# c-zhou/oatk

Hardware: AMD Instinct MI355X
Metric: HiFi Gbases/s through syncasm (syncmer+syncerr) at k=1001 s=31 (higher is better)
Workload: dtype u64

## Files before the change

### oatk_amd/csrc/api.hip

```cpp
#include <hip/hip_runtime.h>
#include <rocprim/device/device_radix_sort.hpp>
#include <rocprim/device/device_scan.hpp>
#include <rocprim/device/device_transform.hpp>
#include <stdio.h>
#include <stdlib.h>
#include <string.h>
#include <time.h>
#include <sys/mman.h>
#include <mutex>
#include <string>
#include <thread>
#include <utility>
#include <vector>

#include "../../include/oatk_hip.h"
#include "devmem.hpp"
#include "common.hpp"
#include "scan_hpc.hpp"
#include "scan_syncmer.hpp"
#include "scan_syncmer_fast.hpp"
#include "kmer_hash.hpp"
#include "count.hpp"

struct oatk_hip_ctx {
    int device = 0;
    int n_cu = 256;
    hipStream_t stream = nullptr;
    std::string err;
    bool timing = false;
    hipEvent_t ev[OATK_T_COUNT_ + 1][2];
    bool ev_used[OATK_T_COUNT_ + 1];
    float ms[OATK_T_COUNT_];
    uint64_t hash_mask = ~0ULL;
    bool force_general = false;
    void *staging = nullptr;
    uint64_t staging_cap = 0;
    void *staging_raw = nullptr;
    uint64_t staging_raw_size = 0;
    bool ra_two_pass = false;
    int list_cap = 0;
    uint64_t import_reserve = 1u << 20;
    int ec_cap_t0 = 0, ec_cap_t1 = 0;

    const uint8_t *d_seq = nullptr;
    const uint64_t *d_off = nullptr;
    const uint32_t *d_len = nullptr;
    DevBuf in_seq, in_off, in_len;
    uint64_t n_reads = 0, seq_bytes = 0, sid0 = 0;
    int K = 0, S = 0;
    bool scanned = false, counted = false;
    bool slots_packed = false;

    DevBuf hoco_l, n_scm, n_nn, n_lrl, ho_rl, hoco_s, nbits;
    DevBuf nn_key, lrl_key, lrl_val, nn_key2, lrl_key2, lrl_val2;
    DevBuf raw_lo, raw_smer, raw_mpos, shard_cnt;
    uint32_t region_cap = 0;
    DevBuf counters;
    uint32_t nn_cap = 0, lrl_cap = 0;
    uint64_t n_occ = 0, tot_nn = 0, tot_lrl = 0, n_scm_total = 0;
    uint32_t retries = 0, collisions = 0;
    bool nn_sorted_in_2 = false, lrl_sorted_in_2 = false;

    DevBuf n_scm64, scm_off, pos_hash, pos_lo, pos_smer, pos_mpos, pos_kid;
    DevBuf key_hash, key_sorted, iota, perm, head, head_idx, newclus, clus_id, bad_head, tag, tmp_perm, flags, kloc, smer_sorted, slot_rec, scm_loc;
    DevBuf scm_h, scm_s, scm_cov, scm_occ_off, scm_occ;
    DevBuf tmp;
    struct EcState *ec = nullptr;
    struct ConsState *cons = nullptr;
    struct IngState *ing = nullptr;
    struct InfState *inf = nullptr;
    struct StatState *stat = nullptr;
    struct AgState *ag = nullptr;
    struct OvlState *ovl = nullptr;
    struct RaState *ra = nullptr;
    struct RcState *rc = nullptr;
    struct MultiState *multi = nullptr;
};

#define CK(call)                                                                                   \
    do {                                                                                           \
        hipError_t e_ = (call);                                                                    \
        if (e_ != hipSuccess) {                                                                    \
            ctx->err = std::string(#call) + ": " + hipGetErrorString(e_);                          \
            return OATK_E_NODEV;                                                                   \
        }                                                                                          \
    } while (0)
static bool debug_refuse(oatk_hip_ctx *ctx, int bit, const char *what)
{
    const char *e = getenv("OATK_DEBUG_REFUSE");
    if (!e || !(atoi(e) & bit)) return false;
    ctx->err = std::string(what) + ": refused on request (OATK_DEBUG_REFUSE)";
    return true;
}

static void t_begin(oatk_hip_ctx *ctx, int which)
{
    if (!ctx->timing) return;
    (void) hipEventRecord(ctx->ev[which][0], ctx->stream);
}
static void t_end(oatk_hip_ctx *ctx, int which)
{
    if (!ctx->timing) return;
    (void) hipEventRecord(ctx->ev[which][1], ctx->stream);
    ctx->ev_used[which] = true;
}
static void t_collect(oatk_hip_ctx *ctx, int first, int last)
{
    if (!ctx->timing) return;
    (void) hipStreamSynchronize(ctx->stream);
    for (int i = first; i <= last; ++i) {
        ctx->ms[i] = 0.f;
        if (ctx->ev_used[i]) (void) hipEventElapsedTime(&ctx->ms[i], ctx->ev[i][0], ctx->ev[i][1]);
        ctx->ev_used[i] = false;
    }
}

#include "api_prim.inc"
#include "api_ec.inc"
#include "api_graph.inc"
#include "api_cons.inc"
#include "api_ovl.inc"
#include "api_align.inc"
#include "api_ingest.inc"
#include "api_bam.inc"
#include "api_inflate.inc"
#include "api_stat.inc"
#include "api_multi.inc"
#include "api_multi_tail.inc"
#include "api_racov.inc"
#include "api_multiplex.inc"

static void staging_free(oatk_hip_ctx *ctx)
{
    if (!ctx->staging) return;
    if (ctx->staging_raw) { (void) hipHostUnregister(ctx->staging); munmap(ctx->staging_raw, ctx->staging_raw_size); }
    else (void) hipHostFree(ctx->staging);
    ctx->staging = ctx->staging_raw = nullptr, ctx->staging_cap = ctx->staging_raw_size = 0;
}

extern "C" {

int oatk_hip_abi_version(void) { return OATK_HIP_ABI_VERSION; }

int oatk_hip_device_count(void)
{
    int n = 0;
    if (hipGetDeviceCount(&n) != hipSuccess) return 0;
    return n;
}

int oatk_hip_max_k(void) { return 8192 - 16 * oatk::SYN_NT - 16 - 64; }

oatk_hip_ctx *oatk_hip_create(int device)
{
    int n = 0;
    if (hipGetDeviceCount(&n) != hipSuccess || device < 0 || device >= n) return nullptr;
    if (hipSetDevice(device) != hipSuccess) return nullptr;
    oatk_hip_ctx *ctx = new oatk_hip_ctx();
    ctx->device = device;
    { int cu = 0; if (hipDeviceGetAttribute(&cu, hipDeviceAttributeMultiprocessorCount, device) == hipSuccess && cu > 0) ctx->n_cu = cu; }
    if (hipStreamCreateWithFlags(&ctx->stream, hipStreamNonBlocking) != hipSuccess) { delete ctx; return nullptr; }
    for (int i = 0; i <= OATK_T_COUNT_; ++i) {
        (void) hipEventCreate(&ctx->ev[i][0]);
        (void) hipEventCreate(&ctx->ev[i][1]);
        ctx->ev_used[i] = false;
    }
    memset(ctx->ms, 0, sizeof(ctx->ms));
    return ctx;
}

void oatk_hip_destroy(oatk_hip_ctx *ctx)
{
    if (!ctx) return;
    (void) hipSetDevice(ctx->device);
    (void) hipStreamSynchronize(ctx->stream);
    ec_state_free(ctx);
    cons_state_free(ctx);
    ing_state_free(ctx);
    inf_state_free(ctx);
    stat_state_free(ctx);
    ag_state_free(ctx);
    ovl_state_free(ctx);
    ra_state_free(ctx);
    rc_state_free(ctx);
    multi_state_free(ctx);
    for (int i = 0; i <= OATK_T_COUNT_; ++i) {
        (void) hipEventDestroy(ctx->ev[i][0]);
        (void) hipEventDestroy(ctx->ev[i][1]);
    }
    staging_free(ctx);
    (void) hipStreamDestroy(ctx->stream);
    delete ctx;
}

int oatk_hip_mem_pool(oatk_hip_ctx *ctx, uint64_t warm_bytes)
{
    if (!ctx) return OATK_E_NODEV;
    { const char *e = getenv("OATK_POOL"); if (e && e[0] == '0') return OATK_OK; }
    CK(hipSetDevice(ctx->device));
    if (ctx->device < 0 || ctx->device >= 64) return OATK_E_ARG;
    ChunkPool *pl;
    {
        std::unique_lock<std::mutex> lk(g_pool_mu);
        pl = g_pool[ctx->device];
        if (!pl) {
            int vmm = 0;
            if (hipDeviceGetAttribute(&vmm, hipDeviceAttributeVirtualMemoryManagementSupported, ctx->device) != hipSuccess || !vmm) { (void) hipGetLastError(); return OATK_OK; }
            pl = new ChunkPool();
            pl->device = ctx->device;
            memset(&pl->prop, 0, sizeof(pl->prop));
            pl->prop.type = hipMemAllocationTypePinned;
            pl->prop.location.type = hipMemLocationTypeDevice;
            pl->prop.location.id = ctx->device;
            memset(&pl->acc, 0, sizeof(pl->acc));
            pl->acc.location = pl->prop.location;
            pl->acc.flags = hipMemAccessFlagsProtReadWrite;
            static bool at_exit = false;
            if (!at_exit) { at_exit = true; atexit(pools_end); }
            pl->on = true;
            g_pool[ctx->device] = pl;
        }
    }
    if (warm_bytes) pl->warm((size_t) warm_bytes);
    return OATK_OK;
}

const char *oatk_hip_last_error(oatk_hip_ctx *ctx) { return ctx? ctx->err.c_str() : "no device context"; }
void *oatk_hip_stream(oatk_hip_ctx *ctx) { return ctx? (void *) ctx->stream : nullptr; }
int oatk_hip_sync(oatk_hip_ctx *ctx)
{
    if (!ctx) return OATK_E_NODEV;
    CK(hipStreamSynchronize(ctx->stream));
    return OATK_OK;
}
int oatk_hip_set_timing(oatk_hip_ctx *ctx, int enable)
{
    if (!ctx) return OATK_E_NODEV;
    ctx->timing = enable != 0;
    return OATK_OK;
}
int oatk_hip_get_timing(oatk_hip_ctx *ctx, float *ms, int n)
{
    if (!ctx) return OATK_E_NODEV;
    for (int i = 0; i < n && i < OATK_T_COUNT_; ++i) ms[i] = ctx->ms[i];
    return OATK_OK;
}
int oatk_hip_debug_force_general(oatk_hip_ctx *ctx, int on)
{
    if (!ctx) return OATK_E_NODEV;
    ctx->force_general = on != 0;
    return OATK_OK;
}
int oatk_hip_debug_align_two_pass(oatk_hip_ctx *ctx, int on)
{
    if (!ctx) return OATK_E_NODEV;
    ctx->ra_two_pass = on != 0;
    return OATK_OK;
}
int oatk_hip_debug_list_cap(oatk_hip_ctx *ctx, int cap)
{
    if (!ctx) return OATK_E_NODEV;
    if (cap < 0 || cap > oatk::SYF_LIST) { ctx->err = "oatk_hip_debug_list_cap: 0 <= cap <= 128"; return OATK_E_ARG; }
    ctx->list_cap = cap;
    return OATK_OK;
}
int oatk_hip_debug_hash_mask(oatk_hip_ctx *ctx, uint64_t mask)
{
    if (!ctx) return OATK_E_NODEV;
    ctx->hash_mask = mask;
    return OATK_OK;
}

static void scan_reset_downstream(oatk_hip_ctx *ctx);

static int launch_scan_kernels(oatk_hip_ctx *ctx)
{
    using namespace oatk;
    const uint64_t n = ctx->n_reads;
    CK(hipMemsetAsync(ctx->counters.p, 0, 4 * sizeof(uint32_t), ctx->stream));
    CK(hipMemsetAsync(ctx->shard_cnt.p, 0, oatk::OATK_REC_SHARDS * sizeof(uint32_t), ctx->stream));
    HpcArgs h;
    h.seq = ctx->d_seq, h.off = ctx->d_off, h.len = ctx->d_len, h.sid0 = ctx->sid0;
    h.ho_rl = ctx->ho_rl.as<uint8_t>(), h.hoco_s = ctx->hoco_s.as<uint8_t>(), h.nbits = ctx->nbits.as<uint32_t>();
    h.hoco_l = ctx->hoco_l.as<uint32_t>(), h.n_nn = ctx->n_nn.as<uint32_t>(), h.n_lrl = ctx->n_lrl.as<uint32_t>();
    h.nn_key = ctx->nn_key.as<uint64_t>(), h.lrl_key = ctx->lrl_key.as<uint64_t>(), h.lrl_val = ctx->lrl_val.as<uint32_t>();
    h.nn_cap = ctx->nn_cap, h.lrl_cap = ctx->lrl_cap, h.counters = ctx->counters.as<uint32_t>();
    t_begin(ctx, OATK_T_HPC);
    h.n_reads = (uint32_t) n;
    constexpr int HPC_NW = 4;
    uint64_t hpc_grid = (uint64_t) ctx->n_cu * 8 * 8;
    { const char *ev = getenv("OATK_DEBUG_HPC_GRID"); if (ev && atoi(ev) > 0) hpc_grid = (uint64_t) atoi(ev); }
    if (hpc_grid * HPC_NW > n) hpc_grid = (n + HPC_NW - 1) / HPC_NW;
    unsigned hpc_dyn = 0;
    { const char *ev = getenv("OATK_DEBUG_HPC_LDS"); if (ev && atoi(ev) > 0) hpc_dyn = (unsigned) atoi(ev); }
    hipLaunchKernelGGL((hpc_pack_kernel<HPC_NW>), dim3((unsigned) (hpc_grid? hpc_grid : 1)), dim3(HPC_NW * OATK_WAVE), hpc_dyn, ctx->stream, h);
    t_end(ctx, OATK_T_HPC);

    SynArgs s;
    s.hoco_s = ctx->hoco_s.as<uint8_t>(), s.nbits = ctx->nbits.as<uint32_t>(), s.off = ctx->d_off;
    s.hoco_l = ctx->hoco_l.as<uint32_t>(), s.n_nn = ctx->n_nn.as<uint32_t>(), s.sid0 = ctx->sid0;
    s.K = ctx->K, s.S = ctx->S, s.want_n = 0, s.n_scm = ctx->n_scm.as<uint32_t>(), s.list_cap = ctx->list_cap? ctx->list_cap : SYF_LIST;
    s.rec_hash = nullptr, s.rec_lo = ctx->raw_lo.as<uint64_t>(), s.rec_smer = ctx->raw_smer.as<uint64_t>();
    s.rec_mpos = ctx->raw_mpos.as<uint32_t>(), s.region_cap = ctx->region_cap, s.shard_cnt = ctx->shard_cnt.as<uint32_t>();
    const bool small = ctx->K + 8 * SYN_NT + 8 + 64 <= 4096;
    const int fast_ring = ctx->force_general? 0 : syncmer_fast_ring(ctx->K, ctx->S);
    t_begin(ctx, OATK_T_SYNCMER);
    if (fast_ring == 4096) {
        const dim3 g((unsigned) n), b(SYN_NT);
        unsigned dyn = 0;
        { const char *ev = getenv("OATK_DEBUG_SYNCMER_LDS"); if (ev && atoi(ev) > 0) dyn = (unsigned) atoi(ev); }
#define OATK_SYF_SWITCH(S31) switch ((-(ctx->K - ctx->S)) & 7) { \
            case 0: OATK_SYF_LAUNCH(S31, 0); break; case 1: OATK_SYF_LAUNCH(S31, 1); break; case 2: OATK_SYF_LAUNCH(S31, 2); break; \
            case 3: OATK_SYF_LAUNCH(S31, 3); break; case 4: OATK_SYF_LAUNCH(S31, 4); break; case 5: OATK_SYF_LAUNCH(S31, 5); break; \
            case 6: OATK_SYF_LAUNCH(S31, 6); break; default: OATK_SYF_LAUNCH(S31, 7); break; }
        const bool two_waves = ctx->K - ctx->S < 1024 && getenv("OATK_DEBUG_SYNCMER_NT256") == nullptr;
#define OATK_SYF_LAUNCH(S31, SH) do { if (two_waves) hipLaunchKernelGGL((syncmer_fast_kernel<2048, S31, 128, SH>), g, dim3(128), dyn, ctx->stream, s); \
                                      else hipLaunchKernelGGL((syncmer_fast_kernel<4096, S31, SYN_NT, SH>), g, b, dyn, ctx->stream, s); } while (0)
        if (ctx->S == 31) OATK_SYF_SWITCH(true) else OATK_SYF_SWITCH(false)
#undef OATK_SYF_SWITCH
#undef OATK_SYF_LAUNCH
    }
    else if (small) hipLaunchKernelGGL((syncmer_kernel<8, 4096, false>), dim3((unsigned) n), dim3(SYN_NT), 0, ctx->stream, s);
    else hipLaunchKernelGGL((syncmer_kernel<16, 8192, false>), dim3((unsigned) n), dim3(SYN_NT), 0, ctx->stream, s);
    t_end(ctx, OATK_T_SYNCMER);
    uint32_t n_amb = 0;
    CK(hipMemcpyAsync(&n_amb, ctx->counters.as<uint32_t>(), 4, hipMemcpyDeviceToHost, ctx->stream));
    CK(hipStreamSynchronize(ctx->stream));
    s.want_n = 1;
    t_begin(ctx, OATK_T_SYNCMER_N);
    if (n_amb) {
        if (small) hipLaunchKernelGGL((syncmer_kernel<8, 4096, true>), dim3((unsigned) n), dim3(SYN_NT), 0, ctx->stream, s);
        else hipLaunchKernelGGL((syncmer_kernel<16, 8192, true>), dim3((unsigned) n), dim3(SYN_NT), 0, ctx->stream, s);
    }
    t_end(ctx, OATK_T_SYNCMER_N);
    CK(hipGetLastError());
    return OATK_OK;
}

int oatk_hip_scan(oatk_hip_ctx *ctx, const uint8_t *d_seq, const uint64_t *d_off, const uint32_t *d_len,
                  uint64_t n_reads, uint64_t seq_bytes, uint64_t sid0, int k, int s)
{
    if (!ctx) return OATK_E_NODEV;
    CK(hipSetDevice(ctx->device));
    if (!(s > 0 && s < 32 && k > s) || k > oatk_hip_max_k()) { ctx->err = "k/s out of range for the device scan"; return OATK_E_ARG; }
    if (seq_bytes % OATK_READ_ALIGN || n_reads >= 0xFFFFFFFFULL || sid0 + n_reads > 0xFFFFFFFFULL) { ctx->err = "bad batch geometry"; return OATK_E_ARG; }
    ctx->d_seq = d_seq, ctx->d_off = d_off, ctx->d_len = d_len;
    ctx->n_reads = n_reads, ctx->seq_bytes = seq_bytes, ctx->sid0 = sid0, ctx->K = k, ctx->S = s;
    scan_reset_downstream(ctx);
    ctx->retries = 0, ctx->collisions = 0;
    ctx->n_occ = ctx->tot_nn = ctx->tot_lrl = ctx->n_scm_total = 0;
    if (n_reads == 0) { ctx->scanned = true; return OATK_OK; }

    ENSURE(hoco_l, n_reads * 4); ENSURE(n_scm, n_reads * 4); ENSURE(n_nn, n_reads * 4); ENSURE(n_lrl, n_reads * 4);
    ENSURE(ho_rl, seq_bytes + 64);
    ENSURE(hoco_s, seq_bytes / 4 + 128 + 16 + ctx->import_reserve);
    ENSURE(nbits, seq_bytes / 8 + 128, true);
    ENSURE(counters, 64);
    if (ctx->nn_cap == 0) ctx->nn_cap = 1u << 14;
    if (ctx->lrl_cap == 0) ctx->lrl_cap = 1u << 14;
    const uint32_t NSH = oatk::OATK_REC_SHARDS;
    {
        uint64_t guess = (seq_bytes / 256 + 1024) / NSH + 256;
        if (ctx->region_cap < guess) ctx->region_cap = (uint32_t) guess;
    }
    ENSURE(shard_cnt, NSH * 4);
    uint32_t sc[oatk::OATK_REC_SHARDS];
    uint32_t sc_max = 0;

    for (;;) {
        const size_t raw_n = (size_t) ctx->region_cap * NSH;
        ENSURE(raw_lo, raw_n * 8); ENSURE(raw_smer, raw_n * 8); ENSURE(raw_mpos, raw_n * 4);
        ENSURE(nn_key, (size_t) ctx->nn_cap * 8); ENSURE(nn_key2, (size_t) ctx->nn_cap * 8);
        ENSURE(lrl_key, (size_t) ctx->lrl_cap * 8); ENSURE(lrl_key2, (size_t) ctx->lrl_cap * 8);
        ENSURE(lrl_val, (size_t) ctx->lrl_cap * 4); ENSURE(lrl_val2, (size_t) ctx->lrl_cap * 4);
        int rc = launch_scan_kernels(ctx);
        if (rc) return rc;
        uint32_t c[4];
        CK(hipMemcpyAsync(c, ctx->counters.p, sizeof(c), hipMemcpyDeviceToHost, ctx->stream));
        CK(hipMemcpyAsync(sc, ctx->shard_cnt.p, sizeof(sc), hipMemcpyDeviceToHost, ctx->stream));
        CK(hipStreamSynchronize(ctx->stream));
        bool again = false;
        if (c[0] > ctx->nn_cap) ctx->nn_cap = c[0] + c[0] / 4, again = true;
        if (c[1] > ctx->lrl_cap) ctx->lrl_cap = c[1] + c[1] / 4, again = true;
        uint64_t tot = 0;
        uint32_t mx = 0;
        for (uint32_t i = 0; i < NSH; ++i) { tot += sc[i]; if (sc[i] > mx) mx = sc[i]; }
        sc_max = mx;
        if (mx > ctx->region_cap) ctx->region_cap = mx + mx / 4 + 16, again = true;
        if (tot > 0xFFFFFFF0ULL) { ctx->err = "more than 2^32 syncmer occurrences in one batch"; return OATK_E_ARG; }
        ctx->tot_nn = c[0], ctx->tot_lrl = c[1], ctx->n_occ = tot;
        if (!again) break;
        ++ctx->retries;
        CK(hipMemsetAsync(ctx->nbits.p, 0, ctx->nbits.cap, ctx->stream));
    }
    if (ctx->timing) t_collect(ctx, OATK_T_HPC, OATK_T_SYNCMER_N);

    t_begin(ctx, OATK_T_SCAN_POST);
    ctx->nn_sorted_in_2 = ctx->lrl_sorted_in_2 = false;
    if (ctx->tot_nn > 1) {
        PRIM(rocprim::radix_sort_keys, ctx->nn_key.as<uint64_t>(), ctx->nn_key2.as<uint64_t>(), ctx->tot_nn, 0, 64, ctx->stream);
        ctx->nn_sorted_in_2 = true;
    }
    if (ctx->tot_lrl > 1) {
        PRIM(rocprim::radix_sort_pairs, ctx->lrl_key.as<uint64_t>(), ctx->lrl_key2.as<uint64_t>(), ctx->lrl_val.as<uint32_t>(), ctx->lrl_val2.as<uint32_t>(), ctx->tot_lrl, 0, 64,
             ctx->stream);
        ctx->lrl_sorted_in_2 = true;
    }
    {
        ENSURE(n_scm64, (n_reads + 1) * 8); ENSURE(scm_off, (n_reads + 1) * 8);
        unsigned nb = (unsigned) ((n_reads + 1 + 255) / 256);
        hipLaunchKernelGGL(widen_kernel, dim3(nb), dim3(256), 0, ctx->stream, ctx->n_scm.as<uint32_t>(), ctx->n_scm64.as<uint64_t>(), n_reads);
        PRIM(rocprim::exclusive_scan, ctx->n_scm64.as<uint64_t>(), ctx->scm_off.as<uint64_t>(), (uint64_t) 0, n_reads + 1, rocprim::plus<uint64_t>(), ctx->stream);
    }
    t_end(ctx, OATK_T_SCAN_POST);

    {
        size_t n = ctx->n_occ? ctx->n_occ : 1;
        ENSURE(pos_hash, n * 8); ENSURE(pos_lo, n * 8); ENSURE(pos_smer, n * 8); ENSURE(pos_mpos, n * 4);
        ENSURE(key_hash, n * 8); ENSURE(iota, n * 4); ENSURE(slot_rec, n * 32);
    }
    if (ctx->n_occ) {
        oatk::KmerHashArgs kh;
        kh.hoco_s = ctx->hoco_s.as<uint8_t>(), kh.off = ctx->d_off, kh.sid0 = ctx->sid0;
        kh.raw_lo = ctx->raw_lo.as<uint64_t>(), kh.raw_smer = ctx->raw_smer.as<uint64_t>(), kh.raw_mpos = ctx->raw_mpos.as<uint32_t>();
        kh.shard_cnt = ctx->shard_cnt.as<uint32_t>(), kh.region_cap = ctx->region_cap;
        kh.scm_off = ctx->scm_off.as<uint64_t>(), kh.hash_mask = ctx->hash_mask;
        kh.pos_hash = ctx->pos_hash.as<uint64_t>(), kh.pos_lo = ctx->pos_lo.as<uint64_t>(), kh.pos_smer = ctx->pos_smer.as<uint64_t>();
        kh.pos_mpos = ctx->pos_mpos.as<uint32_t>(), kh.key_hash = ctx->key_hash.as<uint64_t>(), kh.iota = ctx->iota.as<uint32_t>();
        kh.slot_rec = ctx->slot_rec.as<uint4>(), kh.K = ctx->K;
        t_begin(ctx, OATK_T_KMER_HASH);
        hipLaunchKernelGGL(oatk::kmer_hash_kernel, dim3((sc_max + KMH_WG_REC - 1) / KMH_WG_REC, NSH), dim3(KMH_WG_WAVES * 64), oatk::kmh_lds_bytes(ctx->K), ctx->stream, kh);
        t_end(ctx, OATK_T_KMER_HASH);
    }
    CK(hipGetLastError());
    CK(hipStreamSynchronize(ctx->stream));
    if (ctx->timing) { t_collect(ctx, OATK_T_SCAN_POST, OATK_T_COUNT_PLACE); t_collect(ctx, OATK_T_KMER_HASH, OATK_T_KMER_HASH); }
    ctx->scanned = true;
    ctx->slots_packed = ctx->n_occ != 0;
    return OATK_OK;
}

__global__ void append_rebase_kernel(const uint64_t *src, uint64_t *dst, uint64_t n, uint64_t add)
{
    uint64_t i = (uint64_t) blockIdx.x * blockDim.x + threadIdx.x;
    if (i < n) dst[i] = src[i] + add;
}
__global__ void append_iota_kernel(uint32_t *iota, uint64_t first, uint64_t n)
{
    uint64_t i = (uint64_t) blockIdx.x * blockDim.x + threadIdx.x;
    if (i < n) iota[first + i] = (uint32_t) (first + i);
}

static void scan_reset_downstream(oatk_hip_ctx *ctx)
{
    ctx->scanned = ctx->counted = false;
    ctx->slots_packed = false;
    if (ctx->ec) ctx->ec->done = ctx->ec->marked = ctx->ec->graph_resident = ctx->ec->global = false;
    if (ctx->cons) ctx->cons->done = false;
    if (ctx->ag) ctx->ag->done = false;
    if (ctx->ovl) ctx->ovl->done = false;
    if (ctx->ra) ctx->ra->done = false;
    if (ctx->multi) ctx->multi->merged = ctx->multi->ec_done = false;
}

int oatk_hip_device(oatk_hip_ctx *ctx) { return ctx? ctx->device : -1; }

int oatk_hip_d2d(oatk_hip_ctx *ctx, void *d_dst, const void *d_src, uint64_t bytes)
{
    if (!ctx) return OATK_E_NODEV;
    if (bytes == 0) return OATK_OK;
    CK(hipSetDevice(ctx->device));
    CK(hipMemcpyAsync(d_dst, d_src, bytes, hipMemcpyDeviceToDevice, ctx->stream));
    CK(hipStreamSynchronize(ctx->stream));
    return OATK_OK;
}

int oatk_hip_scan_begin(oatk_hip_ctx *ctx, uint64_t sid0, int k, int s)
{
    if (!ctx) return OATK_E_NODEV;
    CK(hipSetDevice(ctx->device));
    if (!(s > 0 && s < 32 && k > s) || k > oatk_hip_max_k()) { ctx->err = "k/s out of range for the device scan"; return OATK_E_ARG; }
    scan_reset_downstream(ctx);
    ctx->d_seq = nullptr, ctx->d_off = nullptr, ctx->d_len = nullptr;
    ctx->n_reads = 0, ctx->seq_bytes = 0, ctx->sid0 = sid0, ctx->K = k, ctx->S = s;
    ctx->retries = 0, ctx->collisions = 0;
    ctx->n_occ = ctx->tot_nn = ctx->tot_lrl = ctx->n_scm_total = 0;
    ctx->nn_sorted_in_2 = ctx->lrl_sorted_in_2 = false;
    ctx->scanned = true;
    return OATK_OK;
}

#define KEEP(buf, bytes, used)                                                                     \
    do {                                                                                           \
        if (!ctx->buf.grow_keep((bytes), (used), ctx->stream)) {                                   \
            ctx->err = "hipMalloc failed for " #buf " (append)";                                   \
            return OATK_E_NOMEM;                                                                   \
        }                                                                                          \
    } while (0)

static int append_ensure(oatk_hip_ctx *ctx, uint64_t nr, uint64_t sb, uint64_t occ, uint64_t nn, uint64_t lrl)
{
    const uint64_t n0 = ctx->n_reads, b0 = ctx->seq_bytes, o0 = ctx->n_occ;
    KEEP(in_off, (nr + 1) * 8, n0 * 8);
    KEEP(hoco_l, nr * 4 + 4, n0 * 4); KEEP(n_scm, nr * 4 + 4, n0 * 4); KEEP(n_nn, nr * 4 + 4, n0 * 4); KEEP(n_lrl, nr * 4 + 4, n0 * 4);
    KEEP(ho_rl, sb + 64, b0);
    KEEP(hoco_s, sb / 4 + 128 + 16 + ctx->import_reserve, b0 / 4 + 64);
    KEEP(scm_off, (nr + 1) * 8, (n0 + 1) * 8);
    KEEP(pos_hash, occ * 8 + 8, o0 * 8); KEEP(pos_lo, occ * 8 + 8, o0 * 8); KEEP(pos_smer, occ * 8 + 8, o0 * 8); KEEP(pos_mpos, occ * 4 + 4, o0 * 4);
    KEEP(key_hash, occ * 8 + 8, o0 * 8); KEEP(iota, occ * 4 + 4, o0 * 4);
    KEEP(nn_key, nn * 8 + 8, ctx->tot_nn * 8); KEEP(lrl_key, lrl * 8 + 8, ctx->tot_lrl * 8); KEEP(lrl_val, lrl * 4 + 4, ctx->tot_lrl * 4);
    return OATK_OK;
}

int oatk_hip_scan_reserve(oatk_hip_ctx *ctx, uint64_t seq_bytes, uint64_t n_reads, uint64_t n_occ)
{
    if (!ctx) return OATK_E_NODEV;
    CK(hipSetDevice(ctx->device));
    if (!ctx->scanned || ctx->d_seq) { ctx->err = "oatk_hip_scan_reserve: call oatk_hip_scan_begin first"; return OATK_E_STATE; }
    seq_bytes = (seq_bytes + 63) & ~63ULL;
    if (pool_of_current_device()) {
        const uint64_t sb = ctx->seq_bytes + seq_bytes;
        if (!ctx->ho_rl.reserve(sb + 64, ctx->seq_bytes, ctx->stream) || !ctx->hoco_s.reserve(sb / 4 + 128 + 16 + ctx->import_reserve, ctx->seq_bytes / 4 + 64, ctx->stream)) {
            ctx->err = "oatk_hip_scan_reserve: no address range for the batch";
            return OATK_E_NOMEM;
        }
        return OATK_OK;
    }
    return append_ensure(ctx, ctx->n_reads + n_reads, ctx->seq_bytes + seq_bytes, ctx->n_occ + n_occ, ctx->tot_nn, ctx->tot_lrl);
}

int oatk_hip_scan_append(oatk_hip_ctx *ctx, oatk_hip_ctx *src)
{
    if (!ctx || !src) return OATK_E_NODEV;
    CK(hipSetDevice(ctx->device));
    if (ctx == src || ctx->device != src->device) { ctx->err = "oatk_hip_scan_append: the piece must be another handle on the same device"; return OATK_E_ARG; }
    if (!ctx->scanned || ctx->d_seq) { ctx->err = "oatk_hip_scan_append: call oatk_hip_scan_begin first"; return OATK_E_STATE; }
    if (!src->scanned) { ctx->err = "oatk_hip_scan_append: the piece holds no scan"; return OATK_E_STATE; }
    const uint64_t n0 = ctx->n_reads, n1 = src->n_reads, b0 = ctx->seq_bytes, b1 = src->seq_bytes, o0 = ctx->n_occ, o1 = src->n_occ;
    if (n1 == 0) return OATK_OK;
    if (src->K != ctx->K || src->S != ctx->S) { ctx->err = "oatk_hip_scan_append: the piece was scanned with another k / s"; return OATK_E_ARG; }
    if (src->sid0 != ctx->sid0 + n0) { ctx->err = "oatk_hip_scan_append: the piece's first read id must continue the batch"; return OATK_E_ARG; }
    if (n0 + n1 >= 0xFFFFFFFFULL || o0 + o1 > 0xFFFFFFF0ULL) { ctx->err = "oatk_hip_scan_append: batch too large"; return OATK_E_ARG; }
    scan_reset_downstream(ctx);
    ctx->scanned = true;
    { int rc = append_ensure(ctx, n0 + n1, b0 + b1, o0 + o1, ctx->tot_nn + src->tot_nn, ctx->tot_lrl + src->tot_lrl); if (rc) return rc; }
    if (hipStreamSynchronize(src->stream) != hipSuccess) { ctx->err = "oatk_hip_scan_append: the piece's stream failed"; return OATK_E_NODEV; }
    hipStream_t st = ctx->stream;
    auto d2d = [&](void *dst, const void *from, size_t bytes) { return bytes? hipMemcpyAsync(dst, from, bytes, hipMemcpyDeviceToDevice, st) : hipSuccess; };
    CK(d2d(ctx->ho_rl.as<uint8_t>() + b0, src->ho_rl.p, b1));
    CK(d2d(ctx->hoco_s.as<uint8_t>() + b0 / 4, src->hoco_s.p, b1 / 4 + 64));
    CK(d2d(ctx->hoco_l.as<uint32_t>() + n0, src->hoco_l.p, n1 * 4)); CK(d2d(ctx->n_scm.as<uint32_t>() + n0, src->n_scm.p, n1 * 4));
    CK(d2d(ctx->n_nn.as<uint32_t>() + n0, src->n_nn.p, n1 * 4)); CK(d2d(ctx->n_lrl.as<uint32_t>() + n0, src->n_lrl.p, n1 * 4));
    hipLaunchKernelGGL(append_rebase_kernel, grid256(n1), dim3(256), 0, st, src->d_off, ctx->in_off.as<uint64_t>() + n0, n1, b0);
    hipLaunchKernelGGL(append_rebase_kernel, grid256(n1 + 1), dim3(256), 0, st, src->scm_off.as<uint64_t>(), ctx->scm_off.as<uint64_t>() + n0, n1 + 1, o0);
    if (o1) {
        CK(d2d(ctx->pos_hash.as<uint64_t>() + o0, src->pos_hash.p, o1 * 8)); CK(d2d(ctx->pos_lo.as<uint64_t>() + o0, src->pos_lo.p, o1 * 8));
        CK(d2d(ctx->pos_smer.as<uint64_t>() + o0, src->pos_smer.p, o1 * 8)); CK(d2d(ctx->pos_mpos.as<uint32_t>() + o0, src->pos_mpos.p, o1 * 4));
        CK(d2d(ctx->key_hash.as<uint64_t>() + o0, src->key_hash.p, o1 * 8));
        hipLaunchKernelGGL(append_iota_kernel, grid256(o1), dim3(256), 0, st, ctx->iota.as<uint32_t>(), o0, o1);
    }
    CK(d2d(ctx->nn_key.as<uint64_t>() + ctx->tot_nn, src->nn_sorted_in_2? src->nn_key2.p : src->nn_key.p, src->tot_nn * 8));
    CK(d2d(ctx->lrl_key.as<uint64_t>() + ctx->tot_lrl, src->lrl_sorted_in_2? src->lrl_key2.p : src->lrl_key.p, src->tot_lrl * 8));
    CK(d2d(ctx->lrl_val.as<uint32_t>() + ctx->tot_lrl, src->lrl_sorted_in_2? src->lrl_val2.p : src->lrl_val.p, src->tot_lrl * 4));
    CK(hipGetLastError());
    CK(hipStreamSynchronize(st));
    ctx->d_off = ctx->in_off.as<uint64_t>();
    ctx->n_reads = n0 + n1, ctx->seq_bytes = b0 + b1, ctx->n_occ = o0 + o1;
    ctx->tot_nn += src->tot_nn, ctx->tot_lrl += src->tot_lrl;
    ctx->retries += src->retries;
    return OATK_OK;
}

int oatk_hip_scan_host(oatk_hip_ctx *ctx, const uint8_t *h_seq, const uint64_t *h_off, const uint32_t *h_len,
                       uint64_t n_reads, uint64_t seq_bytes, uint64_t sid0, int k, int s)
{
    if (!ctx) return OATK_E_NODEV;
    CK(hipSetDevice(ctx->device));
    ENSURE(in_seq, seq_bytes + 64); ENSURE(in_off, (n_reads + 1) * 8); ENSURE(in_len, (n_reads + 1) * 4);
    if (seq_bytes) CK(hipMemcpyAsync(ctx->in_seq.p, h_seq, seq_bytes, hipMemcpyHostToDevice, ctx->stream));
    if (n_reads) {
        CK(hipMemcpyAsync(ctx->in_off.p, h_off, n_reads * 8, hipMemcpyHostToDevice, ctx->stream));
        CK(hipMemcpyAsync(ctx->in_len.p, h_len, n_reads * 4, hipMemcpyHostToDevice, ctx->stream));
    }
    return oatk_hip_scan(ctx, ctx->in_seq.as<uint8_t>(), ctx->in_off.as<uint64_t>(), ctx->in_len.as<uint32_t>(), n_reads, seq_bytes, sid0, k, s);
}

int oatk_hip_count(oatk_hip_ctx *ctx)
{
    using namespace oatk;
    if (!ctx) return OATK_E_NODEV;
    if (!ctx->scanned) { ctx->err = "count before scan"; return OATK_E_STATE; }
    CK(hipSetDevice(ctx->device));
    ctx->counted = false;
// ... 239 lines not shown
```

### oatk_amd/csrc/scan_hpc.hpp

```cpp
#pragma once
#include <type_traits>
#include "common.hpp"

namespace oatk {

constexpr int HPC_BPT = 16;

struct HpcSqueezeTab {
    uint8_t v[4096];
    constexpr HpcSqueezeTab() : v()
    {
        for (int m = 0; m < 16; ++m)
            for (int c = 0; c < 256; ++c) {
                int out = 0, k = 0;
                for (int i = 0; i < 4; ++i)
                    if (m >> i & 1) out |= ((c >> (2 * i)) & 3) << (6 - 2 * k), ++k;
                v[m << 8 | c] = (uint8_t) out;
            }
    }
};
__device__ const HpcSqueezeTab hpc_squeeze_tab = HpcSqueezeTab();

struct HpcGapTab {
    uint64_t v[256];
    constexpr HpcGapTab() : v()
    {
        for (int m = 0; m < 256; ++m) {
            uint64_t out = 0;
            int k = 0, prev = -1;
            for (int i = 0; i < 8; ++i)
                if (m >> i & 1) {
                    if (prev >= 0) out |= (uint64_t) (i - prev - 1) << (8 * k);
                    prev = i, ++k;
                }
            v[m] = out;
        }
    }
};
__device__ const HpcGapTab hpc_gap_tab = HpcGapTab();

struct HpcArgs {
    const uint8_t *seq;
    const uint64_t *off;
    const uint32_t *len;
    uint64_t sid0;
    uint8_t *ho_rl;
    uint8_t *hoco_s;
    uint32_t *nbits;
    uint32_t *hoco_l, *n_nn, *n_lrl;
    uint64_t *nn_key;
    uint64_t *lrl_key;
    uint32_t *lrl_val;
    uint32_t nn_cap, lrl_cap;
    uint32_t *counters;
    uint32_t n_reads;
};

template <int CTRL, int ROW_MASK = 0xf>
__device__ __forceinline__ uint32_t hpc_dpp(uint32_t old, uint32_t src)
{
    return (uint32_t) __builtin_amdgcn_update_dpp((int) old, (int) src, CTRL, ROW_MASK, 0xf, false);
}

__device__ __forceinline__ uint32_t wave_incl_sum_dpp(uint32_t v, uint32_t lane)
{
    (void) lane;
    v += hpc_dpp<0x111>(0u, v);
    v += hpc_dpp<0x112>(0u, v);
    v += hpc_dpp<0x114>(0u, v);
    v += hpc_dpp<0x118>(0u, v);
    v += hpc_dpp<0x142, 0xa>(0u, v);
    v += hpc_dpp<0x143, 0xc>(0u, v);
    return v;
}
__device__ __forceinline__ int32_t wave_incl_max_dpp(int32_t v, uint32_t lane)
{
    (void) lane;
    int32_t t;
    t = (int32_t) hpc_dpp<0x111>((uint32_t) v, (uint32_t) v); v = t > v? t : v;
    t = (int32_t) hpc_dpp<0x112>((uint32_t) v, (uint32_t) v); v = t > v? t : v;
    t = (int32_t) hpc_dpp<0x114>((uint32_t) v, (uint32_t) v); v = t > v? t : v;
    t = (int32_t) hpc_dpp<0x118>((uint32_t) v, (uint32_t) v); v = t > v? t : v;
    t = (int32_t) hpc_dpp<0x142, 0xa>((uint32_t) v, (uint32_t) v); v = t > v? t : v;
    t = (int32_t) hpc_dpp<0x143, 0xc>((uint32_t) v, (uint32_t) v); v = t > v? t : v;
    return v;
}

template <int NW>
__global__ __launch_bounds__(NW * OATK_WAVE) void hpc_pack_kernel(HpcArgs a)
{
    constexpr int NT = NW * OATK_WAVE;
    constexpr int TILE = OATK_WAVE * HPC_BPT;
    constexpr int RING = 2 * TILE;
    __shared__ uint4 ring_rl4_all[NW][RING / 16];
    __shared__ uint4 ring_hs4_all[NW][RING / 64];
    __shared__ uint8_t lut[256];
    __shared__ uint4 sq4[256];
    __shared__ uint64_t gap8[256];
    __shared__ uint32_t s_rare[NW][2];

    const uint32_t tid = threadIdx.x, lane = tid & 63;
    const uint32_t wid = (uint32_t) __builtin_amdgcn_readfirstlane((int) (tid >> 6));
    uint4 *ring_rl4 = ring_rl4_all[wid], *ring_hs4 = ring_hs4_all[wid];
    uint8_t *ring_rl = (uint8_t *) ring_rl4;
    uint32_t *ring_hs = (uint32_t *) ring_hs4;

    for (uint32_t i = tid; i < 256; i += NT) {
        lut[i] = (uint8_t) nt4_code(i);
        sq4[i] = ((const uint4 *) hpc_squeeze_tab.v)[i];
        gap8[i] = hpc_gap_tab.v[i];
    }
    const uint8_t *sq = (const uint8_t *) sq4;
    for (uint32_t i = tid; i < NW * RING / 64; i += NT) (&ring_hs4_all[0][0])[i] = make_uint4(0, 0, 0, 0);
    for (uint32_t i = tid; i < NW * RING / 16; i += NT) (&ring_rl4_all[0][0])[i] = make_uint4(0, 0, 0, 0);
    __syncthreads();
    auto sync = [&]() __attribute__((always_inline)) {
        __builtin_amdgcn_fence(__ATOMIC_RELEASE, "workgroup");
        __builtin_amdgcn_wave_barrier();
        __builtin_amdgcn_fence(__ATOMIC_ACQUIRE, "workgroup");
    };

    for (uint32_t r = blockIdx.x * NW + wid; r < a.n_reads; r += gridDim.x * NW) {
    const uint64_t o = a.off[r];
    const uint32_t L = a.len[r];
    const uint64_t sid = a.sid0 + r;
    const uint8_t *in = a.seq + o;
    uint8_t *out_rl = a.ho_rl + o;
    uint8_t *out_hs = a.hoco_s + (o >> 2);
    uint32_t *out_nb = a.nbits + (o >> 5);
    if (lane == 0) s_rare[wid][0] = 0, s_rare[wid][1] = 0;

    auto flush = [&](uint32_t g0, uint32_t g1) {
        const uint32_t n_rl = (g1 - g0) * 4u, n_item = n_rl + (g1 - g0);
        for (uint32_t it = lane; it < n_item; it += OATK_WAVE) {
            if (it < n_rl) {
                const uint32_t idx = g0 * 4u + it;
                ((uint4 *) out_rl)[idx] = ring_rl4[idx & (RING / 16 - 1)];
                ring_rl4[idx & (RING / 16 - 1)] = make_uint4(0, 0, 0, 0);
            } else {
                const uint32_t g = g0 + (it - n_rl);
                uint4 v = ring_hs4[g & (RING / 64 - 1)];
                ring_hs4[g & (RING / 64 - 1)] = make_uint4(0, 0, 0, 0);
                v.x = __builtin_bswap32(v.x), v.y = __builtin_bswap32(v.y), v.z = __builtin_bswap32(v.z), v.w = __builtin_bswap32(v.w);
                ((uint4 *) out_hs)[g] = v;
            }
        }
    };
    auto rare = [&](uint32_t h, uint32_t p0, uint32_t rl, uint32_t c) {
        if (rl > 255u) {
            uint32_t idx = atomicAdd(&a.counters[1], 1u);
            if (idx < a.lrl_cap) a.lrl_key[idx] = sid << 32 | h, a.lrl_val[idx] = rl - 1u;
            atomicAdd(&s_rare[wid][1], 1u);
        }
        if (c == 4u) {
            atomicOr(&out_nb[h >> 5], 1u << (h & 31u));
            uint32_t idx = atomicAdd(&a.counters[0], 1u);
            if (idx < a.nn_cap) a.nn_key[idx] = sid << 32 | p0;
            atomicAdd(&s_rare[wid][0], 1u);
        }
    };

    uint32_t nstart = 0;
    int32_t last_start = -1;
    uint32_t flushed = 0;

    uint4 vnext = make_uint4(0, 0, 0, 0);
    uint32_t upnext = 0;
    if (lane * HPC_BPT < L) vnext = *(const uint4 *) (in + lane * HPC_BPT);

    auto tile = [&](const uint32_t t0, auto full_tag, auto hp_tag) __attribute__((always_inline)) {
        constexpr bool FULL = decltype(full_tag)::value, HP = decltype(hp_tag)::value;
        const uint32_t b0 = t0 + lane * HPC_BPT;
        const uint4 v = vnext;
        uint32_t upb = hpc_dpp<0x138>(0u, v.w >> 24);
        if (lane == 0) upb = upnext;
        if (b0 + TILE < L) vnext = *(const uint4 *) (in + b0 + TILE);
        if (lane == 0 && b0 + TILE <= L) upnext = in[b0 + TILE - 1];
        const int nvalid = FULL? HPC_BPT : b0 < L? (int) (L - b0 < (uint32_t) HPC_BPT? L - b0 : (uint32_t) HPC_BPT) : 0;

        uint32_t smask = 0;
        uint32_t pf = 0;
        uint32_t cx = 0, cy = 0, up = 0;
        bool slow = !FULL && nvalid > 0 && nvalid < HPC_BPT;
        const bool wave_slow = !FULL && __ballot(slow) != 0;
        if (nvalid == HPC_BPT && wave_slow) slow = true;
        else if (nvalid == HPC_BPT) {
            constexpr uint32_t TL = 0x01000000u, TH = 0x02000303u;
            constexpr uint32_t EL = 0x43FF41FFu, EH = 0x47FF5554u;
            const uint32_t wds[4] = {v.x, v.y, v.z, v.w};
            uint32_t diff = 0, f = 0;
            uint32_t pk[4];
#pragma unroll
            for (int q = 0; q < 4; ++q) {
                const uint32_t sel = wds[q] & 0x07070707u;
                diff |= (wds[q] & 0xDFDFDFDFu) ^ __builtin_amdgcn_perm(EH, EL, sel);
                const uint32_t c = ((wds[q] >> 1) ^ (wds[q] >> 2)) & 0x03030303u;
                pk[q] = c * 0x01041040u;
            }
            f = __builtin_amdgcn_perm(__builtin_amdgcn_perm(pk[3], pk[2], 0x00000703u), __builtin_amdgcn_perm(pk[1], pk[0], 0x00000703u), 0x05040100u);
            uint32_t cu = 0;
            if (HP || b0) {
                const uint32_t sel = upb & 7u;
                cu = __builtin_amdgcn_perm(TH, TL, sel) & 3u;
                diff |= ((upb & 0xDFu) ^ __builtin_amdgcn_perm(EH, EL, sel)) & 0xFFu;
            }
            pf = f << 2 | cu;
            uint32_t s = f ^ pf;
            s = (s | s >> 1) & 0x55555555u;
            s = (s | s >> 1) & 0x33333333u;
            s = (s | s >> 2) & 0x0F0F0F0Fu;
            s = (s | s >> 4) & 0x00FF00FFu;
            smask = (s | s >> 8) & 0xFFFFu;
            if (!HP && b0 == 0) smask |= 1u;
            slow = diff != 0;
        }
        if (slow) {
            cx = cy = 0;
            up = 7u;
            const uint32_t wds[4] = {v.x, v.y, v.z, v.w};
#pragma unroll
            for (int b = 0; b < 8; ++b) {
                cx |= (uint32_t) lut[(wds[b >> 2] >> (8 * (b & 3))) & 0xffu] << (4 * b);
                cy |= (uint32_t) lut[(wds[2 + (b >> 2)] >> (8 * (b & 3))) & 0xffu] << (4 * b);
            }
            if (nvalid < HPC_BPT) {
                const uint64_t keep = (1ULL << (4 * nvalid)) - 1ULL;
                uint64_t cc = ((uint64_t) cy << 32 | cx);
                cc = (cc & keep) | (0x7777777777777777ULL & ~keep);
                cx = (uint32_t) cc, cy = (uint32_t) (cc >> 32);
            }
            if (HP || b0 > 0) up = lut[upb & 0xffu];
            const uint32_t px = cx << 4 | up, py = cy << 4 | cx >> 28;
            const uint32_t dx = cx ^ px, dy = cy ^ py;
            const uint32_t LOW = 0x11111111u;
            uint32_t sx = (dx | dx >> 1 | dx >> 2) & LOW, sy = (dy | dy >> 1 | dy >> 2) & LOW;
            sx |= (cx >> 2) & ~(cx >> 1) & ~cx & LOW;
            sy |= (cy >> 2) & ~(cy >> 1) & ~cy & LOW;
            sx &= ~((cx >> 2) & (cx >> 1) & cx) & LOW;
            sy &= ~((cy >> 2) & (cy >> 1) & cy) & LOW;
            auto squeeze = [](uint32_t s) -> uint32_t {
                s = (s | s >> 3) & 0x03030303u;
                s = (s | s >> 6) & 0x000f000fu;
                s = (s | s >> 12) & 0x000000ffu;
                return s;
            };
            smask = squeeze(sx) | squeeze(sy) << 8;
            uint64_t x = (((uint64_t) cy << 32 | cx) << 4 | up) & 0x3333333333333333ULL;
            x = (x | x >> 2) & 0x0f0f0f0f0f0f0f0fULL;
            x = (x | x >> 4) & 0x00ff00ff00ff00ffULL;
            x = (x | x >> 8) & 0x0000ffff0000ffffULL;
            pf = (uint32_t) (x | x >> 16);
        }
        const uint32_t cnt = __builtin_popcount(smask);
        const int32_t lpos = smask? (int32_t) (b0 + 31 - __builtin_clz(smask)) : -1;
        const uint32_t icnt = wave_incl_sum_dpp(cnt, lane);
        const int32_t imax = __ballot(lpos < 0)? wave_incl_max_dpp(lpos, lane) : lpos;
        const uint32_t tot = (uint32_t) __builtin_amdgcn_readlane((int) icnt, 63);
        const int32_t wmax = __builtin_amdgcn_readlane(imax, 63), tmax = wmax > last_start? wmax : last_start;
        sync();
        int32_t ls = (int32_t) hpc_dpp<0x138>((uint32_t) -1, (uint32_t) imax);
        if (lane == 0) ls = -1;
        const uint32_t n = nstart + icnt - cnt;
        if (last_start > ls) ls = last_start;
        if (smask) {
            const uint64_t cls64 = (uint64_t) cy << 32 | cx;
            uint32_t fin = smask;
            if (!HP && b0 == 0) fin &= ~1u;
            uint32_t special = 0;
            if (slow) {
                const uint64_t prevc = cls64 << 4 | up;
                const uint64_t is4 = (prevc >> 2) & ~(prevc >> 1) & ~prevc & 0x1111111111111111ULL;
                uint64_t spread = fin;
                spread = (spread | spread << 24) & 0x000000ff000000ffULL;
                spread = (spread | spread << 12) & 0x000f000f000f000fULL;
                spread = (spread | spread << 6) & 0x0303030303030303ULL;
                spread = (spread | spread << 3) & 0x1111111111111111ULL;
                special = (is4 & spread) != 0;
            }
            if (fin) {
                const uint32_t t0b = sq[(fin & 0xFu) << 8 | (pf & 0xFFu)];
                const uint32_t t1b = sq[(fin & 0xF0u) << 4 | ((pf >> 8) & 0xFFu)];
                const uint32_t t2b = sq[(fin & 0xF00u) | ((pf >> 16) & 0xFFu)];
                const uint32_t t3b = sq[(fin & 0xF000u) >> 4 | pf >> 24];
                const uint32_t c1 = (uint32_t) __builtin_popcount(fin & 0xFu), c2 = (uint32_t) __builtin_popcount(fin & 0xFFu),
                               c3 = (uint32_t) __builtin_popcount(fin & 0xFFFu);
                const uint32_t rv = t0b << 24 | t1b << (24u - 2u * c1) | t2b << (24u - 2u * c2) | t3b << (24u - 2u * c3);
                const uint32_t hfirst = n - 1u + (!HP && b0 == 0? 1u : 0u);
                const uint32_t off = (hfirst & 15u) * 2u;
                const uint64_t sh = ((uint64_t) rv << 32) >> off;
                const uint32_t w0 = (hfirst & (RING - 1)) >> 4;
                const uint32_t hiw = (uint32_t) (sh >> 32), low = (uint32_t) sh;
                if (hiw) atomicOr(&ring_hs[w0], hiw);
                if (low) atomicOr(&ring_hs[(w0 + 1) & (RING / 16 - 1)], low);
                const uint32_t bf = (uint32_t) __builtin_ctz(smask);
                uint32_t first = 0;
                if ((fin >> bf) & 1u) {
                    const uint32_t rl = (uint32_t) ((int32_t) (b0 + bf) - ls);
                    first = (rl > 256u? 256u : rl) - 1u;
                    special |= rl > 255u;
                }
                {
                    const uint32_t slo = smask & 0xFFu, shi = smask >> 8;
                    uint64_t glo = gap8[slo], ghi = gap8[shi];
                    const uint32_t between = (uint32_t) (__ffs((int) shi) + __clz((int) slo)) - 25u;
                    glo |= slo? first : 0u;
                    ghi |= slo? (shi? between : 0u) : first;
                    const uint32_t h0 = n - 1u;
                    const uint32_t sl = (h0 & 3u) * 8u, shh = sl + (uint32_t) __builtin_popcount(slo) * 8u;
                    const uint32_t t = shh & 31u, q4 = (shh >> 5) * 4u;
                    const uint64_t L0 = (uint64_t) (uint32_t) glo << sl, L1 = (glo >> 32) << sl;
                    const uint64_t H0 = (uint64_t) (uint32_t) ghi << t, H1 = (ghi >> 32) << t;
                    const uint32_t l0 = (uint32_t) L0, l1 = (uint32_t) (L0 >> 32) | (uint32_t) L1, l2 = (uint32_t) (L1 >> 32);
                    const uint32_t g0 = (uint32_t) H0, g1 = (uint32_t) (H0 >> 32) | (uint32_t) H1, g2 = (uint32_t) (H1 >> 32);
                    const uint32_t ab = h0 & (uint32_t) (RING - 1) & ~3u;
                    if (ab <= (uint32_t) RING - 24u) {
                        uint32_t *pl = (uint32_t *) ((char *) ring_rl4 + ab), *ph = (uint32_t *) ((char *) ring_rl4 + ab + q4);
                        atomicOr(pl, l0), atomicOr(pl + 1, l1), atomicOr(pl + 2, l2);
                        atomicOr(ph, g0), atomicOr(ph + 1, g1), atomicOr(ph + 2, g2);
                    } else {
                        auto at = [&](uint32_t b) -> uint32_t * { return (uint32_t *) ((char *) ring_rl4 + (b & (uint32_t) (RING - 1))); };
                        atomicOr(at(ab), l0), atomicOr(at(ab + 4u), l1), atomicOr(at(ab + 8u), l2);
                        atomicOr(at(ab + q4), g0), atomicOr(at(ab + q4 + 4u), g1), atomicOr(at(ab + q4 + 8u), g2);
                    }
                }
            }
            if (special) {
                uint32_t k2 = 0;
                int32_t p2 = ls;
                for (int b = 0; b < HPC_BPT; ++b) {
                    if ((smask >> b) & 1u) {
                        const int32_t i = (int32_t) (b0 + b);
                        if (i > 0) {
                            const uint32_t pc = b? (uint32_t) (cls64 >> (4 * (b - 1))) & 7u : up;
                            rare(n + k2 - 1u, (uint32_t) p2, (uint32_t) (i - p2), pc);
                        }
                        p2 = i;
                        ++k2;
                    }
                }
            }
        }
        sync();
        nstart += tot;
        last_start = tmax;
        const uint32_t done = nstart? (nstart - 1u) >> 6 : 0u;
        flush(flushed, done);
        flushed = done;
    };
    for (uint32_t t0 = 0; t0 < L; t0 += TILE) {
        if (t0 && t0 + TILE <= L) tile(t0, std::true_type(), std::true_type()); else tile(t0, std::false_type(), std::false_type());
    }
    if (lane == 0 && nstart) {
        const uint32_t h = nstart - 1u, rl = L - (uint32_t) last_start, c = lut[in[L - 1]];
        ring_rl[h & (RING - 1)] = (uint8_t) ((rl > 256u? 256u : rl) - 1u);
        if (c & 3u & (c < 4u? 3u : 0u)) atomicOr(&ring_hs[(h & (RING - 1)) >> 4], (c & 3u) << (30u - 2u * (h & 15u)));
        rare(h, (uint32_t) last_start, rl, c);
    }
    sync();
    flush(flushed, (nstart + 63u) >> 6);
    if (lane == 0) {
        a.hoco_l[r] = nstart;
        a.n_nn[r] = s_rare[wid][0];
        a.n_lrl[r] = s_rare[wid][1];
    }
    sync();
    }
}

}
```

Measured before the change: 421.4.

## Pad partial HPC tiles with last base and derive predecessor via DPP on packed codes

The HPC pack kernel now pads the tail of partial tiles with the read's final base, so partial tiles take the fast bit-packed path instead of the LUT slow path. It computes the previous-base code by shifting packed codes across lanes with DPP and alignbit, and carries the last byte through a readlane instead of a separate scalar load. It also iterates set bits of the start mask with ctz in the rare-record loop and enlarges the launch grid in proportion to read count. The padding trick depends on a repeated last base never creating a new homopolymer start, and the clamped prefetch address adds index arithmetic.

```diff
diff --git a/oatk_amd/csrc/api.hip b/oatk_amd/csrc/api.hip
--- a/oatk_amd/csrc/api.hip
+++ b/oatk_amd/csrc/api.hip
@@ -289,6 +289,7 @@
     h.n_reads = (uint32_t) n;
     constexpr int HPC_NW = 4;
     uint64_t hpc_grid = (uint64_t) ctx->n_cu * 8 * 8;
+    { const uint64_t by_reads = n / (HPC_NW * 4), most = (uint64_t) ctx->n_cu * 8 * 32; if (by_reads > hpc_grid) hpc_grid = by_reads < most? by_reads : most; }
     { const char *ev = getenv("OATK_DEBUG_HPC_GRID"); if (ev && atoi(ev) > 0) hpc_grid = (uint64_t) atoi(ev); }
     if (hpc_grid * HPC_NW > n) hpc_grid = (n + HPC_NW - 1) / HPC_NW;
     unsigned hpc_dyn = 0;
diff --git a/oatk_amd/csrc/scan_hpc.hpp b/oatk_amd/csrc/scan_hpc.hpp
--- a/oatk_amd/csrc/scan_hpc.hpp
+++ b/oatk_amd/csrc/scan_hpc.hpp
@@ -165,27 +165,37 @@
     uint32_t flushed = 0;
 
     uint4 vnext = make_uint4(0, 0, 0, 0);
-    uint32_t upnext = 0;
+    uint32_t upcarry = 0;
     if (lane * HPC_BPT < L) vnext = *(const uint4 *) (in + lane * HPC_BPT);
+    const uint32_t lastb = L? (uint32_t) __builtin_amdgcn_readfirstlane((int) in[L - 1]) : 0u;
+    const uint32_t padw = lastb * 0x01010101u;
+    const uint32_t lim = ((L + 63u) & ~63u) - (uint32_t) HPC_BPT;
 
     auto tile = [&](const uint32_t t0, auto full_tag, auto hp_tag) __attribute__((always_inline)) {
         constexpr bool FULL = decltype(full_tag)::value, HP = decltype(hp_tag)::value;
         const uint32_t b0 = t0 + lane * HPC_BPT;
-        const uint4 v = vnext;
-        uint32_t upb = hpc_dpp<0x138>(0u, v.w >> 24);
-        if (lane == 0) upb = upnext;
-        if (b0 + TILE < L) vnext = *(const uint4 *) (in + b0 + TILE);
-        if (lane == 0 && b0 + TILE <= L) upnext = in[b0 + TILE - 1];
+        uint4 v = vnext;
+        if (FULL || t0 + TILE < L) {
+            const uint32_t nb = b0 + TILE;
+            vnext = *(const uint4 *) (in + (nb < lim? nb : lim));
+        }
         const int nvalid = FULL? HPC_BPT : b0 < L? (int) (L - b0 < (uint32_t) HPC_BPT? L - b0 : (uint32_t) HPC_BPT) : 0;
+        if (!FULL) {
+            uint32_t w[4] = {v.x, v.y, v.z, v.w};
+#pragma unroll
+            for (int q = 0; q < 4; ++q) {
+                const int nv = nvalid - 4 * q;
+                const uint32_t keep = nv >= 4? ~0u : nv > 0? (1u << (8 * nv)) - 1u : 0u;
+                w[q] = (w[q] & keep) | (padw & ~keep);
+            }
+            v = make_uint4(w[0], w[1], w[2], w[3]);
+        }
 
         uint32_t smask = 0;
         uint32_t pf = 0;
         uint32_t cx = 0, cy = 0, up = 0;
-        bool slow = !FULL && nvalid > 0 && nvalid < HPC_BPT;
-        const bool wave_slow = !FULL && __ballot(slow) != 0;
-        if (nvalid == HPC_BPT && wave_slow) slow = true;
-        else if (nvalid == HPC_BPT) {
-            constexpr uint32_t TL = 0x01000000u, TH = 0x02000303u;
+        bool slow;
+        {
             constexpr uint32_t EL = 0x43FF41FFu, EH = 0x47FF5554u;
             const uint32_t wds[4] = {v.x, v.y, v.z, v.w};
             uint32_t diff = 0, f = 0;
@@ -198,13 +208,9 @@
                 pk[q] = c * 0x01041040u;
             }
             f = __builtin_amdgcn_perm(__builtin_amdgcn_perm(pk[3], pk[2], 0x00000703u), __builtin_amdgcn_perm(pk[1], pk[0], 0x00000703u), 0x05040100u);
-            uint32_t cu = 0;
-            if (HP || b0) {
-                const uint32_t sel = upb & 7u;
-                cu = __builtin_amdgcn_perm(TH, TL, sel) & 3u;
-                diff |= ((upb & 0xDFu) ^ __builtin_amdgcn_perm(EH, EL, sel)) & 0xFFu;
-            }
-            pf = f << 2 | cu;
+            uint32_t prevf = hpc_dpp<0x138>(0u, f);
+            if (lane == 0) prevf = ((upcarry >> 1) ^ (upcarry >> 2)) << 30;
+            pf = __builtin_amdgcn_alignbit(f, prevf, 30);
             uint32_t s = f ^ pf;
             s = (s | s >> 1) & 0x55555555u;
             s = (s | s >> 1) & 0x33333333u;
@@ -212,9 +218,13 @@
             s = (s | s >> 4) & 0x00FF00FFu;
             smask = (s | s >> 8) & 0xFFFFu;
             if (!HP && b0 == 0) smask |= 1u;
-            slow = diff != 0;
-        }
+            const bool carry_bad = (HP || t0) && (upcarry & 0xDFu) != ((uint32_t) ((((uint64_t) EH << 32) | EL) >> (8u * (upcarry & 7u))) & 0xFFu);
+            slow = __ballot(diff != 0) != 0 || carry_bad;
+        }
+        uint32_t upb = 0;
         if (slow) {
+            upb = hpc_dpp<0x138>(0u, v.w >> 24);
+            if (lane == 0) upb = upcarry;
             cx = cy = 0;
             up = 7u;
             const uint32_t wds[4] = {v.x, v.y, v.z, v.w};
@@ -251,6 +261,7 @@
             x = (x | x >> 8) & 0x0000ffff0000ffffULL;
             pf = (uint32_t) (x | x >> 16);
         }
+        upcarry = (uint32_t) __builtin_amdgcn_readlane((int) v.w, 63) >> 24;
         const uint32_t cnt = __builtin_popcount(smask);
         const int32_t lpos = smask? (int32_t) (b0 + 31 - __builtin_clz(smask)) : -1;
         const uint32_t icnt = wave_incl_sum_dpp(cnt, lane);
@@ -325,18 +336,18 @@
                 }
             }
             if (special) {
-                uint32_t k2 = 0;
+                uint32_t h2 = n - 1u;
                 int32_t p2 = ls;
-                for (int b = 0; b < HPC_BPT; ++b) {
-                    if ((smask >> b) & 1u) {
-                        const int32_t i = (int32_t) (b0 + b);
-                        if (i > 0) {
-                            const uint32_t pc = b? (uint32_t) (cls64 >> (4 * (b - 1))) & 7u : up;
-                            rare(n + k2 - 1u, (uint32_t) p2, (uint32_t) (i - p2), pc);
-                        }
-                        p2 = i;
-                        ++k2;
+#pragma unroll 1
+                for (uint32_t m = smask; m; m &= m - 1u) {
+                    const uint32_t b = (uint32_t) __builtin_ctz(m);
+                    const int32_t i = (int32_t) (b0 + b);
+                    if (i > 0) {
+                        const uint32_t pc = b? (uint32_t) (cls64 >> (4 * (b - 1))) & 7u : up;
+                        rare(h2, (uint32_t) p2, (uint32_t) (i - p2), pc);
                     }
+                    p2 = i;
+                    ++h2;
                 }
             }
         }
@@ -351,7 +362,7 @@
         if (t0 && t0 + TILE <= L) tile(t0, std::true_type(), std::true_type()); else tile(t0, std::false_type(), std::false_type());
     }
     if (lane == 0 && nstart) {
-        const uint32_t h = nstart - 1u, rl = L - (uint32_t) last_start, c = lut[in[L - 1]];
+        const uint32_t h = nstart - 1u, rl = L - (uint32_t) last_start, c = lut[lastb];
         ring_rl[h & (RING - 1)] = (uint8_t) ((rl > 256u? 256u : rl) - 1u);
         if (c & 3u & (c < 4u? 3u : 0u)) atomicOr(&ring_hs[(h & (RING - 1)) >> 4], (c & 3u) << (30u - 2u * (h & 15u)));
         rare(h, (uint32_t) last_start, rl, c);
```

Measured after the change: 424.1 (median of 6 runs). Within noise of the previous version (+0.7%).
